# DINT-NSDI24/DINT

Hardware: AMD Instinct MI355X
Metric: Mtxn/s + p50/p99 batch latency, TATP (higher is better)
Workload: dtype u64

## Files before the change

dint_amd/csrc/dint_kv.h:

```cpp
#pragma once
#include <cstdlib>
#include <utility>
#include <vector>

#include "dint_kernels.h"
#include "dint_kv_core.h"
#include "state_block.h"
#include "state_image.h"

#define DINT_KV_MAX_TABLES 5
#define DINT_KV_CTL_BYTES (64 + 24 * KV_NLISTS)
#define DINT_KV_TRACE_WORDS ((size_t)DINT_KV_PMAX * 16 + 16 * 8192)
#define DINT_KV_LOAD_OP 0xF0u

struct kv_dev {
  kv_tab tab[DINT_KV_MAX_TABLES];
  dint_mod mod[DINT_KV_MAX_TABLES];
  dint_mod lockmod[DINT_KV_MAX_TABLES];
  uint32_t gk_base[DINT_KV_MAX_TABLES];
  uint32_t n_tables;
  uint32_t shard_index, shard_count;
  uint32_t same_key;
  uint32_t pass_ins[DINT_KV_MAX_TABLES];
};

struct dint_kv_knobs {
  uint32_t coarse_load = 512;
  uint32_t cap = 0;
  uint32_t lcap = 1024;
  uint32_t cap_mult = 64;
  uint32_t rpt = 0;
  uint32_t no_bm = 0;
  uint32_t hot_min = 0;
  uint32_t no_split = 0;
  uint32_t split_min = 65;
  uint32_t split_target = 384;
  uint32_t one_big_kernel = 0;
  uint32_t workers = 96;
  uint32_t part_first = 0;
  uint32_t sb_split_min = 65;
  uint32_t sb_npmax = 128;
  uint32_t sb_workers = 130;
  uint32_t sb_late_grid = 32;
  uint32_t residency = 0;
  uint32_t no_fuse = 0;
  uint32_t no_ahead = 0;
  uint32_t late_grid = 8;
  uint32_t exp_no_late = 0;
  uint32_t late_fat = 0;
  uint32_t late_big = 0;
};

struct dint_kv {
  uint32_t workload = 0;
  uint32_t n_tables = 0;
  uint32_t val_size = 0;
  int force_rounds = 0;
  uint64_t hash_size[DINT_KV_MAX_TABLES] = {0, 0, 0, 0, 0};
  kv_dev h{};
  kv_dev *d_dev = nullptr;
  uint8_t *d_ctl = nullptr;
  uint64_t *d_trace = nullptr;
  size_t entry_bytes[DINT_KV_MAX_TABLES] = {0, 0, 0, 0, 0};
  dint_kv_knobs knobs;
};

static inline uint32_t dint_kv_cap_mult() {
  const char *v = getenv("DINT_KV_CAP_MULT");
  const unsigned long m = v && *v ? strtoul(v, nullptr, 10) : 64ul;
  return (uint32_t)(m < 2 ? 2 : m > 256 ? 256 : m);
}
int dint_kv_create(dint_kv *kv, uint32_t workload, uint64_t n_rows, dint_shard shard, uint32_t pool_entries = 0,
                   uint32_t flags = 0);
void dint_kv_destroy(dint_kv *kv);
std::vector<std::pair<void *, size_t>> dint_kv_regions(dint_kv *kv);
int64_t dint_kv_dump_rows(dint_kv *kv, uint32_t table, uint64_t *keys, uint32_t *vers, uint8_t *vals, uint64_t cap);
int64_t dint_kv_read_locks(dint_kv *kv, uint32_t table, uint32_t *a, uint32_t *b, uint64_t cap);
struct dint_kv_ahead {
  const void *d_req;
  void *d_rep;
  uint32_t n;
  dint_view view;
};
bool dint_kv_ahead_ok(const dint_kv &kv, int load_mode);
bool dint_kv_one_launch(const dint_kv &kv, int load_mode);
void dint_launch_kv(const void *d_req, void *d_rep, uint32_t n, const dint_kv &kv, dint_log log, dint_scratch s,
                    int load_mode, hipStream_t st, hipEvent_t *ev, const dint_view &view = dint_flat_view(),
                    bool part_done = false, const dint_kv_ahead *next = nullptr);
#define DINT_KV_MULTI_MAX 4u
struct dint_kv_pass {
  const void *d_req;
  void *d_rep;
  uint32_t n;
  const dint_kv *kv;
  dint_log log;
  dint_scratch s;
  dint_view view;
};
void dint_launch_kv_multi(const dint_kv_pass *p, uint32_t n_eng, hipStream_t st, bool part_done = false, const dint_kv_pass *next = nullptr);
bool dint_kv_multi_ahead_ok(const dint_kv &kv);
void dint_launch_home_kv(const void *d_req, uint32_t n, const dint_kv &kv, uint8_t *d_home, hipStream_t st);
struct dint_kv_fmt {
  uint32_t msg, type, table, key, val, ver, val_size;
};
dint_kv_fmt dint_kv_format(uint32_t workload);

struct dint_state_scratch {
  unsigned long long *words;
  uint32_t *blk_cnt;
  uint64_t *blk_off;
  uint32_t nb;
  unsigned long long *digest_part;
};
#define DINT_STATE_DIGEST_GRID 2048u
#define DINT_STATE_WORDS 48u
#define DINT_STATE_DIGEST_AT 16u
uint32_t dint_state_blocks(const dint_kv &kv);
void dint_launch_state_digest(const dint_kv &kv, dint_state_scratch s, hipStream_t st);
void dint_launch_state_diff_count(const dint_kv &a, const dint_kv &b, dint_state_scratch s, hipStream_t st);
void dint_launch_state_diff_write(const dint_kv &a, const dint_kv &b, dint_state_scratch s, void *d_records, uint64_t cap, hipStream_t st);
void dint_launch_state_repair_check(const dint_kv &kv, const void *d_records, uint64_t n, dint_state_scratch s, hipStream_t st);
void dint_launch_state_repair(const dint_kv &kv, const void *d_records, uint64_t n, uint32_t pend_set, dint_dev_stats *stats,
                              dint_state_scratch s, hipStream_t st);

#define DINT_STATE_STATS_GRID 2048u
#define DINT_STATE_STATS_WORDS 80u
struct dint_stats_scratch {
  unsigned long long *part;
// ... 147 lines not shown
```

dint_amd/csrc/k_kv.hip:

```cpp
#include "k_kv_dev.h"

dint_kv_fmt dint_kv_format(uint32_t workload) {
  switch (workload) {
    case DINT_WL_STORE: return {53, 0, 0xFFFFFFFFu, 1, 9, 49, 40};
    case DINT_WL_TATP: return {55, 1, 2, 3, 11, 51, 40};
    default: return {23, 1, 2, 3, 11, 19, 8};
  }
}


static inline uint32_t kv_pick_coarse(uint32_t n, uint32_t load) {
  uint64_t c = ((uint64_t)n + load - 1) / load;
  if (c < 1) c = 1;
  if (c > DINT_KV_CMAX) c = DINT_KV_CMAX;
  return (uint32_t)c;
}
static uint32_t kv_env(const char *name, uint32_t dflt) {
  const char *v = getenv(name);
  return v && *v ? (uint32_t)strtoul(v, nullptr, 10) : dflt;
}
static dint_kv_knobs kv_read_knobs() {
  dint_kv_knobs k;
  k.coarse_load = std::min(8192u, std::max(64u, kv_env("DINT_KV_COARSE_LOAD", KVB_T)));
  k.cap = kv_env("DINT_KV_CAP", 0);
  k.lcap = std::min(KVR_LCAP, kv_env("DINT_KV_LCAP", KVR_LCAP));
  k.cap_mult = dint_kv_cap_mult();
  k.rpt = kv_env("DINT_KV_RPT", 0);
  k.no_bm = kv_env("DINT_KV_NO_BM", 0);
  k.hot_min = kv_env("DINT_KV_HOT_MIN", 0);
  k.no_split = kv_env("DINT_KV_NO_SPLIT", 0);
  k.split_min = std::max(65u, kv_env("DINT_KV_SPLIT_MIN", 65u));
  k.split_target = std::min(448u, std::max(8u, kv_env("DINT_KV_SPLIT_TARGET", 384u)));
  k.one_big_kernel = kv_env("DINT_KV_ONE_BIG_KERNEL", 0);
  k.no_ahead = kv_env("DINT_KV_NO_AHEAD", 0);
  k.no_fuse = kv_env("DINT_KV_NO_FUSE", 0);
  k.sb_split_min = kv_env("DINT_KV_SB_SPLIT_MIN", 65u);
  k.sb_late_grid = std::max(1u, std::min(KVB_GRID, kv_env("DINT_KV_SB_LATE_GRID", 32u)));
  k.sb_npmax = std::max(2u, std::min(KSB_NPMAX, kv_env("DINT_KV_SB_NPMAX", 128u)));
  k.sb_workers = kv_env("DINT_KV_SB_WORKERS", k.sb_npmax + 2u);
  if (k.sb_workers) k.sb_workers = std::max(k.sb_workers, k.sb_npmax + 2u);
  k.workers = std::min(1024u, std::max(KVR_NPMAX + 2u, kv_env("DINT_KV_WORKERS", KVW_GRID)));
  k.part_first = kv_env("DINT_KV_PART_FIRST", 0) & 1u;
  k.late_grid = std::min(KVB_GRID, std::max(1u, kv_env("DINT_KV_LATE_GRID", 8u)));
  k.late_big = kv_env("DINT_KV_LATE_BIG", 0);
  k.exp_no_late = kv_env("DINT_EXP_NO_LATE", 0);
  k.late_fat = kv_env("DINT_KV_LATE_FAT", 0);
  return k;
}

static inline bool kv_uses_hot(const dint_kv &kv, int load_mode) {
  return kv.workload != DINT_WL_SMALLBANK && !(kv.force_rounds & 3) && !load_mode && !kv.knobs.no_split;
}
bool dint_kv_one_launch(const dint_kv &kv, int load_mode) {
  return kv_uses_hot(kv, load_mode) && !kv.knobs.one_big_kernel && !kv.knobs.no_fuse;
}
bool dint_kv_ahead_ok(const dint_kv &kv, int load_mode) {
  if (kv.workload == DINT_WL_SMALLBANK) return !load_mode && !kv.knobs.no_ahead && !kv.knobs.no_fuse;
  return kv_uses_hot(kv, load_mode) && !kv.knobs.one_big_kernel && !kv.knobs.no_ahead;
}

static void kv_fill_pass(kv_pass_args &A, const void *d_req, void *d_rep, uint32_t n, const dint_kv &kv, dint_log log,
                         const dint_scratch &s, int load_mode, const dint_view &view, uint32_t tile) {
  const dint_kv_knobs &K = kv.knobs;
  const uint32_t C = kv_pick_coarse(n, K.coarse_load);
  const uint32_t mean = (n + C - 1) / C;
  uint32_t cap = K.cap_mult * mean + 64;
  cap = std::min(cap, (uint32_t)(s.kbins_slots / C));
  cap = std::max(1u, K.cap ? std::min(cap, K.cap) : cap);
  A.req = (const uint8_t *)d_req; A.rep = (uint8_t *)d_rep; A.n = n;
  A.n_tiles = (n + tile - 1) / tile;
  A.kv = kv.d_dev; A.log = log; A.cut = kv_make_cut(C, n); A.cap = cap;
  A.lcap = K.lcap;
  const uint64_t pn = s.kvs.pass_no;
  A.pno = (uint32_t)(pn & 1u);
  A.bin_cnt = s.kvs.bin_cnt[pn & 1]; A.kbins = s.kvs.kbins[pn & 1]; A.ovl = s.kvs.ovl[pn & 1];
  A.big = s.kvs.ctl[pn % 3]; A.big_z = s.kvs.ctl[(pn + 2) % 3];
  A.blk_pub = s.kvs.pub[pn % 3]; A.blk_pub_z = s.kvs.pub[(pn + 2) % 3];
  A.bigrdy = s.kvs.bigrdy;
  A.ovf = s.ovf; A.ovf2 = s.ovf2; A.stats = s.stats;
  A.bigq = s.bigq;
  A.hotpub = s.hotpub;
  A.lateq = s.lateq;
  A.seq = s.pass_seq ? s.pass_seq : 1u;
  A.inv_n = n > 1 ? (uint32_t)((1ull << 32) / n) : 0xFFFFFFFFu;
  A.load_mode = load_mode;
  A.force_flags = kv.force_rounds | (K.no_bm ? 4 : 0) | (int)(K.hot_min << 8);
  A.split_min = kv_uses_hot(kv, load_mode) ? K.split_min : 0xFFFFFFFFu;
  A.split_target = K.split_target;
  A.np_max = KVR_NPMAX;
  A.sb_pieces = 0;
  A.sbx = s.kvs.sbx;
  if (kv.workload == DINT_WL_SMALLBANK && K.sb_split_min && s.kvs.sbx && !(kv.force_rounds & 3) && !load_mode && !K.no_split) {
    A.split_min = std::max(8u, K.sb_split_min);
    A.np_max = K.sb_npmax;
    A.sb_pieces = 1;
  }
  A.has_log = kv.workload != DINT_WL_STORE;
  A.trace = kv.d_trace;
  A.V = view;
}

extern template int kv_piece_residency<DINT_WL_STORE>(int);
extern template int kv_piece_residency<DINT_WL_TATP>(int);
extern template int kv_piece_residency<DINT_WL_SMALLBANK>(int);
extern template void launch_kv_passes<DINT_WL_STORE>(kv_multi_args &, uint32_t, uint32_t, hipStream_t, hipEvent_t *, const dint_kv_knobs &, bool, const kv_multi_args *, uint32_t);
extern template void launch_kv_passes<DINT_WL_TATP>(kv_multi_args &, uint32_t, uint32_t, hipStream_t, hipEvent_t *, const dint_kv_knobs &, bool, const kv_multi_args *, uint32_t);
extern template void launch_kv_passes<DINT_WL_SMALLBANK>(kv_multi_args &, uint32_t, uint32_t, hipStream_t, hipEvent_t *, const dint_kv_knobs &, bool, const kv_multi_args *, uint32_t);

static inline uint32_t kv_pick_rpt(uint32_t n_total, const dint_kv_knobs &K) {
  if (K.rpt == 1 || K.rpt == 2 || K.rpt == 4) return K.rpt;
  return n_total >= 1024u * 1024u ? 4u : n_total >= 256u * 1024u ? 2u : 1u;
}
static inline uint32_t kv_pick_rpt_ahead(uint32_t n, const dint_kv_knobs &K) {
  if (K.rpt == 4 || (K.rpt == 0 && n >= 256u * 1024u)) return 4u;
  return 2u;
}

static void launch_kv_dispatch(uint32_t workload, kv_multi_args &M, uint32_t n_eng, uint32_t rpt, hipStream_t st, hipEvent_t *ev,
                               const dint_kv_knobs &K, bool part_done = false, const kv_multi_args *next = nullptr, uint32_t next_rpt = 0) {
  switch (workload) {
    case DINT_WL_STORE: launch_kv_passes<DINT_WL_STORE>(M, n_eng, rpt, st, ev, K, part_done, next, next_rpt); break;
    case DINT_WL_TATP: launch_kv_passes<DINT_WL_TATP>(M, n_eng, rpt, st, ev, K, part_done, next, next_rpt); break;
    default: launch_kv_passes<DINT_WL_SMALLBANK>(M, n_eng, rpt, st, ev, K, part_done, next, next_rpt); break;
  }
}

void dint_launch_kv(const void *d_req, void *d_rep, uint32_t n, const dint_kv &kv, dint_log log, dint_scratch s,
                    int load_mode, hipStream_t st, hipEvent_t *ev, const dint_view &view, bool part_done, const dint_kv_ahead *next) {
  if (n == 0) return;
  kv_multi_args M;
  memset(&M, 0, sizeof M);
  const uint32_t rpt = kv_pick_rpt(n, kv.knobs), rpt_a = kv_pick_rpt_ahead(n, kv.knobs);
  kv_fill_pass(M.e[0], d_req, d_rep, n, kv, log, s, load_mode, view, part_done ? KVB_T * rpt_a : KV_TB * rpt);
  kv_multi_args N;
  uint32_t next_rpt = 0;
  if (next && next->n && dint_kv_ahead_ok(kv, load_mode)) {
    dint_scratch sn = s;
    sn.kvs.pass_no = s.kvs.pass_no + 1;
    sn.pass_seq = s.pass_seq + 1 >= 0x3FFFFFFFu ? 1u : s.pass_seq + 1;
    next_rpt = kv_pick_rpt_ahead(next->n, kv.knobs);
    memset(&N, 0, sizeof N);
    kv_fill_pass(N.e[0], next->d_req, next->d_rep, next->n, kv, log, sn, load_mode, next->view, KVB_T * next_rpt);
  } else {
    next = nullptr;
  }
  launch_kv_dispatch(kv.workload, M, 1, rpt, st, ev, kv.knobs, part_done, next ? &N : nullptr, next_rpt);
}

void dint_launch_kv_multi(const dint_kv_pass *p, uint32_t n_eng, hipStream_t st, bool part_done, const dint_kv_pass *next) {
  if (n_eng == 0) return;
  kv_multi_args M, N;
  memset(&M, 0, sizeof M);
  uint32_t n_total = 0;
  for (uint32_t k = 0; k < n_eng; k++) n_total += p[k].n;
  const uint32_t rpt = kv_pick_rpt(n_total, p[0].kv->knobs);
  for (uint32_t k = 0; k < n_eng; k++) kv_fill_pass(M.e[k], p[k].d_req, p[k].d_rep, p[k].n, *p[k].kv, p[k].log, p[k].s, 0, p[k].view, KV_TB * rpt);
  uint32_t next_rpt = 0;
  if (next) {
    uint32_t nmax = 0;
    for (uint32_t k = 0; k < n_eng; k++) nmax = std::max(nmax, next[k].n);
    next_rpt = kv_pick_rpt_ahead(nmax, p[0].kv->knobs);
    memset(&N, 0, sizeof N);
    for (uint32_t k = 0; k < n_eng; k++) {
      dint_scratch sn = next[k].s;
      sn.kvs.pass_no = p[k].s.kvs.pass_no + 1;
      sn.pass_seq = p[k].s.pass_seq + 1 >= 0x3FFFFFFFu ? 1u : p[k].s.pass_seq + 1;
      kv_fill_pass(N.e[k], next[k].d_req, next[k].d_rep, next[k].n, *next[k].kv, next[k].log, sn, 0, next[k].view, KVB_T * next_rpt);
    }
  }
// ... 235 lines not shown
```

dint_amd/csrc/k_kv_dev.h:

```cpp
#pragma once
#include <algorithm>
#include <cstddef>
#include <cstdlib>
#include <cstring>
#include <utility>
#include <vector>

#include "../../include/dint_abi.h"
#include "dint_kv.h"
#define KVB_SORT_INLINE
#include "dint_bins.h"

template <int WL> struct Fmt;
template <> struct Fmt<DINT_WL_STORE> {
  static constexpr uint32_t MSG = 53, TYPE = 0, KEY = 1, VAL = 9, VER = 49, VS = 40;
  static constexpr bool HAS_TABLE = false;
  static constexpr uint32_t TABLE = 0;
};
template <> struct Fmt<DINT_WL_TATP> {
  static constexpr uint32_t MSG = 55, TYPE = 1, KEY = 3, VAL = 11, VER = 51, VS = 40;
  static constexpr bool HAS_TABLE = true;
  static constexpr uint32_t TABLE = 2;
};
template <> struct Fmt<DINT_WL_SMALLBANK> {
// ... 2002 lines not shown
            uint32_t pos;
            if (fancy) {
              const int lw = top(mW & below), lwb = top((mW | mB) & below);
              const uint32_t w = wc + (uint32_t)__popcll(mW & below);
              const uint32_t jj = (lw < 0 ? jc : 0u) + (uint32_t)__popcll(mB & below & above(lw));
              const uint64_t mine = q == 0 ? mA[0] : q == 1 ? mA[1] : q == 2 ? mA[2] : mA[3];
              const bool follows = (mine & below & above(lwb)) != 0 || (lwb < 0 && ((af >> q) & 1u));
              pos = w * stride + (cl == 0 ? 0u : cl == 1 ? 3u * jj + (follows ? 1u : 0u) : cl == 2 ? 3u * jj + 2u : stride - 1u);
            } else {
              pos = 2u * (vc + (uint32_t)__popcll(mV & below)) + (cl ? 1u : 0u);
            }
            if (valid) Rpos[p] = (uint16_t)pos;
            const int tw = top(mW), twb = top(mW | mB);
            wc += (uint32_t)__popcll(mW);
            jc = (tw < 0 ? jc : 0u) + (uint32_t)__popcll(mB & above(tw));
            if (twb >= 0) af = 0;
#pragma unroll
            for (uint32_t i = 0; i < 4; i++) af |= (mA[i] & above(twb)) ? 1u << i : 0u;
            vc += (uint32_t)__popcll(mV);
          }
        }
      }
    }
    __syncthreads();
    for (uint32_t j = 0; j < ntile; j++) {
      const uint32_t p = j * KVB_T + t;
      const uint32_t pos = p < m ? Rpos[p] : 0xFFFFu;
      if (pos != 0xFFFFu) atomicOr(&Rbits[pos >> 5], 1u << (pos & 31));
    }
    {
      uint32_t mx = mylen;
      for (int d = 32; d > 0; d >>= 1) mx = max(mx, (uint32_t)__shfl_xor(mx, d, 64));
      if (lane == 0) Sred[wave] = mx;
      __syncthreads();
      tot = 0;
      for (uint32_t w = 0; w < KVB_W; w++) tot = max(tot, Sred[w]);
    }
    for (uint32_t rw = 0; rw * 32 < tot; rw++) {
      for (uint32_t bits = Rbits[rw]; bits; bits &= bits - 1) {
        const uint32_t r = rw * 32 + (uint32_t)__ffs((int)bits) - 1;
        nrounds++;
        for (uint32_t j = 0; j < ntile; j++) {
          const uint32_t p = j * KVB_T + t;
          if (p < m && Rpos[p] == r) {
            const uint64_t cur = Sk[p];
            const uint32_t gk = kv_cut_gk((uint32_t)(cur >> sh_g), bin, cut), table = kv_table_of(kv, gk);
            kv_do_request<WL>(rep + dint_view_off(V, k_idx(cur), F::MSG), k_type(cur), table, k_q(cur),
                              (uint64_t)(gk - kv->gk_base[table]), kv, stats);
          }
        }
        __builtin_amdgcn_fence(__ATOMIC_SEQ_CST, "workgroup");
        __syncthreads();
      }
    }
    }
    if (wtr && t == 0) { wtr[14] += nrounds; wtr[15] += 1; }
    KVB_STAMP(13);
    __builtin_amdgcn_fence(__ATOMIC_SEQ_CST, "workgroup");
    __syncthreads();
  }
#undef KVB_STAMP
}

#define KVR_LCAP 1024u
#define KVR_F 64u
#define KVR_NPMAX 64u
struct kvr_lds {
  uint4 rec[KVR_LCAP];
  uint32_t hist[KVR_F];
  uint32_t cur[KVR_F];
  uint32_t off[KVR_F + 1];
  uint32_t bigoff[KVR_F];
  uint2 chs[KVR_F];
  uint32_t nch;
  uint32_t cflag[KVR_F];
  uint64_t ckey[KVR_F], hrec[KVR_F];
};
__device__ static inline uint32_t kv_piece_of(uint32_t idx, uint32_t np, uint32_t inv_n) {
  const uint32_t p = (uint32_t)(((uint64_t)idx * np * inv_n) >> 32);
  return p < np ? p : np - 1;
}
#define KVQ_W 3u
enum : uint32_t { KVQ_SUB = 0, KVQ_PIECE = 1, KVQ_REM = 2, KVQ_SOLO = 3 };

__device__ static inline void kv_list_items(const kv_pass_args &A, uint32_t b, const kvr_lds &L, const uint2 *Sbig) {
  const uint32_t t = threadIdx.x & 63u;
  const uint2 bs = Sbig[t];
  uint32_t target = A.split_target;
  if (A.V.seg_cap) {
    uint32_t live = t < A.V.n_seg ? min(A.V.seg_cap, *(const uint32_t *)(A.V.cnt + (size_t)t * A.V.cnt_stride)) : 0u, tot;
    (void)wave_excl_scan_u32(live, &tot);
    if (tot < A.n) target = max(8u, (uint32_t)(((uint64_t)target * max(tot, 1u)) / A.n));
  }
  const uint32_t np0 = (bs.y + target - 1) / target;
  const bool hot = bs.y >= A.split_min && np0 <= A.np_max;
  const uint32_t np = hot ? np0 : 0u;
  const uint32_t nent = bs.y ? (np > 1 ? np + 1 : 1u) : 0u;
  uint32_t tot, at = wave_excl_scan_u32(nent, &tot);
  uint32_t base = 0;
  if (t == 0 && tot) base = atomicAdd(&A.big[3], tot);
  base = (uint32_t)__builtin_amdgcn_readfirstlane((int)base);
  at += base;
  const uint32_t bin = b + A.cut.P * t;
  if (nent && !hot) {
    kv_st_agent(A.bigq + KVQ_W * (size_t)at, make_uint4(bin, bs.x, bs.y, KVQ_SUB));
  } else if (nent) {
    uint64_t hk = L.ckey[t], hr = L.hrec[t];
    if (A.sb_pieces) {
      using F = Fmt<DINT_WL_SMALLBANK>;
      const uint32_t sh_g = 16 + A.cut.ibits;
      uint64_t smp[8];
#pragma unroll
      for (uint32_t j = 0; j < 8; j++) smp[j] = kv_ld_agent(&A.ovf[bs.x + (uint32_t)(((uint64_t)(2 * j + 1) * bs.y) >> 4)]);
      uint32_t best = 0, bj = 0;
#pragma unroll
      for (uint32_t j = 0; j < 8; j++) {
        uint32_t c = 0;
#pragma unroll
        for (uint32_t i = 0; i < 8; i++) c += (smp[i] >> sh_g) == (smp[j] >> sh_g) && pay_q(kv_rec_pay(smp[i])) == pay_q(kv_rec_pay(smp[j]));
        if (c > best) { best = c; bj = j; }
      }
      hr = smp[0];
#pragma unroll
      for (uint32_t j = 1; j < 8; j++) if (j == bj) hr = smp[j];
      const uint32_t hidx = (uint32_t)(hr >> 16) & (uint32_t)((1ull << A.cut.ibits) - 1ull);
      hk = ld_u64(A.rep + dint_view_off(A.V, hidx, F::MSG) + F::KEY);
    }
    for (uint32_t p = 0; p < nent; p++) {
      const uint32_t kind = np == 1 ? KVQ_SOLO : (p < np ? KVQ_PIECE : KVQ_REM);
      uint4 *q = A.bigq + KVQ_W * (size_t)(at + p);
      kv_st_agent(q, make_uint4(bin, bs.x, bs.y, kind | (p << 2) | (np << 10)));
      kv_st_agent(q + 1, make_uint4((uint32_t)hk, (uint32_t)(hk >> 32), at, 0u));
      kv_st_agent(q + 2, make_uint4((uint32_t)hr, (uint32_t)(hr >> 32), 0u, 0u));
    }
  }
  asm volatile("s_waitcnt vmcnt(0)" ::: "memory");
  for (uint32_t p = 0; p < nent; p++)
    if (at + p < DINT_KV_BIGQ_MAX) __hip_atomic_store(&A.bigrdy[at + p], A.seq, __ATOMIC_RELAXED, __HIP_MEMORY_SCOPE_AGENT);
  asm volatile("s_waitcnt vmcnt(0)" ::: "memory");
  if (t == 0) atomicAdd(&A.big[6], 1u);
}

template <int WL, uint32_t NT>
__device__ static inline void kv_coarse_bin(const kv_pass_args &A, const kv_dev *kv, uint32_t coarse, uint8_t *lds_raw,
                                            uint2 *Sbig ,
                                            uint32_t cnt, const uint4 &r0, const uint4 &r1, uint64_t *tr) {
  kvr_lds &L = *(kvr_lds *)lds_raw;
  const uint32_t t = threadIdx.x, lane = t & 63, wave = t >> 6;
  const kv_cut &cut = A.cut;
  const uint32_t C = cut.P, cap = A.cap, sh = 16 + cut.ibits;
  const uint32_t idx_mask = (uint32_t)((1ull << cut.ibits) - 1ull);
  const uint4 *__restrict__ recs = A.kbins + (size_t)coarse * cap;
  if (cnt == 0) {
    if (t == 0) atomicAdd(&A.big[6], 1u);
    return;
  }
  const uint32_t n_in = min(cnt, cap);
  const uint32_t novl = cnt > cap ? A.big[1] : 0u;
  if (t == 0) A.bin_cnt[coarse] = 0;
  auto for_each_record = [&](auto &&f) {
    if (t < n_in) f(r0);
    if (t + NT < n_in) f(r1);
    for (uint32_t k0 = 2 * NT; k0 < n_in; k0 += 8 * NT) {
      uint4 q4[8];
#pragma unroll
      for (uint32_t j = 0; j < 8; j++) {
// ... 277 lines not shown
      if (lane == 0) { H.Lq[q][wave] = ml; H.Aq[q][wave] = ma; }
    }
  }
  __syncthreads();
  uint32_t ev_below = 0, nW = 0;
#pragma unroll
  for (uint32_t wv = 0; wv < KVB_W; wv++) {
    const uint64_t m = H.Bw[wv];
    nW += (uint32_t)__popcll(m);
    ev_below += (uint32_t)__popcll(wv < wave ? m : (wv == wave ? m & lanemask_lt() : 0ull));
  }
  if (H.gbad || nW > KVG_MAXW) return false;
  uint8_t *msg = rep + dint_view_off(V, my_idx, F::MSG);
  for (uint32_t e = 0; e <= nW; e++) {
    if (isR && ev_below == e) {
      kv_hdr Hh;
      kv_hdr_load(Hh, ie);
      const kv_res r = kv_apply<kv_dev_mem>(tb, bucket, Hh, KV_ACT_GET, my_key, msg + F::VAL, 0, blockIdx.x);
      if (r.ok) st_u32(msg + F::VER, r.ver);
      msg[F::TYPE] = (uint8_t)(WL == DINT_WL_STORE ? (r.ok ? 3 : 7) : (r.ok ? 4 : 6));
    }
    __builtin_amdgcn_fence(__ATOMIC_SEQ_CST, "workgroup");
    __syncthreads();
    if (isW && ev_below == e) {
      kv_hdr Hh;
      kv_hdr_load(Hh, ie);
      const uint32_t act = is_set(my_type) ? KV_ACT_SET : is_ins(my_type) ? KV_ACT_INS : KV_ACT_DEL;
      const kv_res r = kv_apply<kv_dev_mem>(tb, bucket, Hh, act, my_key, msg + F::VAL, 0, blockIdx.x);
      uint32_t code;
      if (WL == DINT_WL_STORE) code = my_type == 1 ? (r.ok ? 5 : 7) : 8;
      else code = my_type == 12 ? 15 : my_type == 13 ? 16 : my_type == 18 ? 20 : my_type == 19 ? 21 : my_type == 22 ? 25 : 26;
      if (!r.ok) {
        if (act == KV_ACT_INS) atomicAdd(&stats->pool_exhausted, 1ULL);
        else if (WL != DINT_WL_STORE) atomicAdd(&stats->missing_keys, 1ULL);
      }
      msg[F::TYPE] = (uint8_t)code;
    }
    __builtin_amdgcn_fence(__ATOMIC_SEQ_CST, "workgroup");
    __syncthreads();
  }
  if (WL == DINT_WL_TATP) {
    const uint32_t lockw = H.lockw;
    if (v && (my_type == 1 || my_type == 2)) {
      int last = -1;
#pragma unroll
      for (uint32_t wv = 0; wv < KVB_W; wv++) {
        const uint64_t m = H.Lq[my_q][wv], mb = wv < wave ? m : (wv == wave ? m & lanemask_lt() : 0ull);
        if (mb) last = (int)(wv * 64 + 63 - __clzll((long long)mb));
      }
      const uint32_t seen = last >= 0 ? (uint32_t)((H.Aq[my_q][last >> 6] >> (last & 63)) & 1ull) : (lockw >> (8 * my_q)) & 0xFFu;
      msg[F::TYPE] = (uint8_t)(my_type == 1 ? (seen ? 8 : 7) : 9);
    }
    if (t < 4) {
      int last = -1;
      for (uint32_t wv = 0; wv < KVB_W; wv++)
        if (H.Lq[t][wv]) last = (int)(wv * 64 + 63 - __clzll((long long)H.Lq[t][wv]));
      if (last >= 0) {
        const uint32_t fin = (uint32_t)((H.Aq[t][last >> 6] >> (last & 63)) & 1ull);
        if (fin != ((lockw >> (8 * t)) & 0xFFu)) KV_ST(uint8_t, ie + KV_LOCKB_OFF + t, (uint8_t)fin);
      }
    }
  }
  __builtin_amdgcn_fence(__ATOMIC_SEQ_CST, "workgroup");
  __syncthreads();
  return true;
}
template <int WL>
__device__ __forceinline__ static int kv_solo_item(uint8_t *rep, const kv_cut cut2, const kv_dev *kv, const uint4 d,
                                                   const uint64_t *__restrict__ ovf, uint64_t *__restrict__ ovf2,
                                                   dint_dev_stats *__restrict__ stats, int force_rounds, const dint_view V, uint8_t *lds_raw,
                                                   uint32_t *src, uint32_t *off, uint32_t *cnt, uint64_t *ttr,
                                                   bool preloaded = false ) {
  using F = Fmt<WL>;
  kvh_lds &H = *(kvh_lds *)lds_raw;
  const uint32_t t = threadIdx.x, lane = t & 63, wave = t >> 6;
  const uint32_t h = d.z;
  const uint32_t sh_g = 16 + cut2.ibits, sh_k = 7 + cut2.ibits, idx_mask = (uint32_t)((1ull << cut2.ibits) - 1ull);
  *src = 0; *off = d.y; *cnt = h;
  if (h > KVB_T) return 1;
  auto is_set = [](uint32_t type) -> bool { return WL == DINT_WL_STORE ? type == 1 : (type == 12 || type == 13); };
  auto is_ins = [](uint32_t type) -> bool { return WL == DINT_WL_STORE ? type == 2 : (type == 18 || type == 19); };
  auto is_del = [](uint32_t type) -> bool { return WL == DINT_WL_TATP && (type == 22 || type == 23); };
  __syncthreads();
  if (!preloaded) H.all[t] = t < h ? kv_sort_key(kv_ld_agent(&ovf[d.y + t]), cut2) : ~0ull;
  if (t == 0) { H.bad = 0; H.best = 0; H.bestg = 0; H.dupf = 0; }
  __syncthreads();
  {
    uint32_t N = 64;
    while (N < h) N <<= 1;
    kvb_sort_blocked<1>(H.all, N);
  }
  const uint64_t w = H.all[t];
  const bool valid = t < h;
  const uint64_t prevw = t ? H.all[t - 1] : 0;
  const bool head_k = valid && (t == 0 || (prevw >> sh_k) != (w >> sh_k));
  const bool head_g = valid && (t == 0 || (prevw >> sh_g) != (w >> sh_g));
  const uint64_t mk = __ballot(head_k), mg = __ballot(head_g);
  if (lane == 0) { H.Bw[wave] = mk; H.Bl[wave] = mg; }
  __syncthreads();
  auto next_head = [&](const uint64_t *M) -> uint32_t {
    uint32_t nxt = h;
    for (uint32_t wv = wave; wv < KVB_W && nxt == h; wv++) {
      uint64_t mm = M[wv];
      if (wv == wave) mm &= ~((2ull << lane) - 1ull);
      if (mm) nxt = wv * 64 + (uint32_t)__ffsll((unsigned long long)mm) - 1;
    }
    return nxt;
  };
  if (head_k) atomicMax(&H.best, ((next_head(H.Bw) - t) << 16) | t);
  if (head_g) atomicMax(&H.bestg, ((next_head(H.Bl) - t) << 16) | t);
  __syncthreads();
  const uint32_t L = H.best >> 16, P = H.best & 0xFFFFu;
  uint32_t Gs = H.bestg & 0xFFFFu, Ge = Gs + (H.bestg >> 16);
  if (L > 64) {
    Gs = 0;
    for (uint32_t wv = 0; wv < KVB_W; wv++) {
      uint64_t mm = H.Bl[wv];
      if (wv * 64 > P) break;
      if (wv == (P >> 6)) mm &= (2ull << (P & 63)) - 1ull;
      if (mm) Gs = wv * 64 + 63 - (uint32_t)__clzll((long long)mm);
    }
    Ge = h;
    for (uint32_t wv = P >> 6; wv < KVB_W && Ge == h; wv++) {
      uint64_t mm = H.Bl[wv];
      if (wv == (P >> 6)) mm &= ~((2ull << (P & 63)) - 1ull);
      if (mm) Ge = wv * 64 + (uint32_t)__ffsll((unsigned long long)mm) - 1;
    }
  }
  auto rest = [&](uint32_t lo, uint32_t len) -> int {
    const uint32_t c_rem = h - len;
    if (c_rem == 0) return 0;
    __syncthreads();
    if (valid && (t < lo || t >= lo + len)) H.rem[t < lo ? t : t - len] = w;
    if (t >= c_rem) H.rem[t] = ~0ull;
    __builtin_amdgcn_fence(__ATOMIC_SEQ_CST, "workgroup");
    if (kv_rem_chunks<WL>(rep, cut2, kv, d.x, H.rem, c_rem, H, stats, force_rounds, V, true)) return 0;
    if (ovf2 && t < c_rem) {
      const uint64_t sw = H.rem[t];
      ovf2[d.y + t] = ((sw >> sh_g) << sh_g) | ((uint64_t)((uint32_t)(sw >> 7) & idx_mask) << 16) | ((uint32_t)sw & 0x7Fu) | (((uint32_t)(sw >> sh_k) & 511u) << 7);
    }
    __builtin_amdgcn_fence(__ATOMIC_SEQ_CST, "workgroup");
    *src = 1; *off = d.y; *cnt = c_rem;
    return 1;
  };
  auto phases = [&]() -> int {
    if (!kv_group_phases<WL>(rep, cut2, kv, d.x, H.all, Gs, Ge, H, stats, V)) return 1;
    return rest(Gs, Ge - Gs);
  };
  if (L <= 64) {
    if (ttr && t == 0) ttr[30] = (uint64_t)(d.w & 0xFFFFu) | (1ull << 17) | ((uint64_t)L << 20) | ((uint64_t)h << 32);
    if (Ge - Gs <= 64) return kv_rem_chunks<WL>(rep, cut2, kv, d.x, H.all, h, H, stats, force_rounds, V, true) ? 0 : 1;
    return phases();
  }
  const uint64_t hw = H.all[P];
  const uint32_t hq = pay_q((uint32_t)hw & 0x7Fu);
  const bool v = valid && t >= P && t < P + L;
  const uint32_t my_idx = (uint32_t)(w >> 7) & idx_mask, my_type = valid ? pay_type((uint32_t)w & 0x7Fu) : 0xFFu;
  if (valid && !v && (w >> sh_g) == (hw >> sh_g) && (kv_struct_op<WL>(my_type) || (kv_lock_op<WL>(my_type) && pay_q((uint32_t)w & 0x7Fu) == hq))) atomicOr(&H.bad, kv_struct_op<WL>(my_type) ? 1u : 2u);
  const uint64_t my_key = v ? ld_u64(rep + dint_view_off(V, my_idx, F::MSG) + F::KEY) : 0;
  if (t == P) H.hkey = my_key;
  const bool setop = v && is_set(my_type), insop = v && is_ins(my_type), delop = v && is_del(my_type);
  const bool lk = v && kv_lock_op<WL>(my_type), aq = v && WL == DINT_WL_TATP && my_type == 1;
  if (v && !(kv_simple_op<WL>(my_type) || kv_struct_op<WL>(my_type))) atomicOr(&H.bad, 4u);
  const uint64_t bev = __ballot(setop || insop || delop), bl = __ballot(lk), ba = __ballot(aq), bst = __ballot(insop || delop);
  if (lane == 0) { H.Bw[wave] = bev; H.Bl[wave] = bl; H.Ba[wave] = ba; }
  if (bst && lane == 0) H.dupf = 1;
  H.idx[t] = my_idx;
// ... 194 lines not shown
  const bool locator = t == 0 && c != 0;
  if (locator) {
    const uint32_t gk = kv_cut_gk((uint32_t)(hrec >> sh_g), d.x, cut2);
    table0 = kv_table_of(kv, gk);
    tb0 = kv->tab[table0];
    bucket0 = (uint64_t)(gk - kv->gk_base[table0]);
    kv_hdr_load(Hd, kv_entry_ptr(tb0, bucket0, KV_INLINE));
  }
  __syncthreads();
  if (do_piece) kvb_sort_blocked_u32<1>(H.key, KVB_T);
  if (locator) {
    const kv_where w = kv_locate(tb0, bucket0, Hd, hkey);
    H.found = w.found; H.link = w.link; H.slot = w.slot; H.ver0 = w.ver; H.table = table0;
    H.la0 = WL == DINT_WL_TATP ? (Hd.lockw >> (8 * hq)) & 0xFFu : 0u;
    if (w.found) {
      const uint8_t *rv = kv_entry_ptr(tb0, bucket0, w.link) + KV_VAL_OFF + w.slot * F::VS;
#pragma unroll
      for (uint32_t k = 0; k < F::VS / 4; k++) H.rowv[k] = KV_LD(uint32_t, rv + 4 * k);
    }
  }
  const uint32_t sk = H.key[t];
  const bool v = do_piece && sk != 0xFFFFFFFFu;
  const uint32_t my_idx = sk >> 9, my_type = v ? H.typ[sk & 511u] : 0xFFu;
  if (v && !kv_simple_op<WL>(my_type)) H.bad = 1;
  const bool wr = v && is_writer(my_type), lk = v && kv_lock_op<WL>(my_type), aq = v && WL == DINT_WL_TATP && my_type == 1;
  const uint64_t bw = __ballot(wr), bl = __ballot(lk), ba = __ballot(aq);
  if (lane == 0) { H.Bw[wave] = bw; H.Bl[wave] = bl; H.Ba[wave] = ba; }
  H.idx[t] = my_idx;
  __syncthreads();
  uint32_t wr_below = 0, wr_tot = 0;
  int lw_below = -1, lw_tot = -1, ll_below = -1, ll_tot = -1;
#pragma unroll
  for (uint32_t w = 0; w < KVB_W; w++) {
    const uint64_t mw = H.Bw[w], ml = H.Bl[w];
    const uint64_t mwb = w < wave ? mw : (w == wave ? mw & lanemask_lt() : 0ull), mlb = w < wave ? ml : (w == wave ? ml & lanemask_lt() : 0ull);
    wr_below += (uint32_t)__popcll(mwb); wr_tot += (uint32_t)__popcll(mw);
    if (mwb) lw_below = (int)(w * 64 + 63 - __clzll((long long)mwb));
    if (mw) lw_tot = (int)(w * 64 + 63 - __clzll((long long)mw));
    if (mlb) ll_below = (int)(w * 64 + 63 - __clzll((long long)mlb));
    if (ml) ll_tot = (int)(w * 64 + 63 - __clzll((long long)ml));
  }
  auto acq_at = [&](int p) -> int { return (int)((H.Ba[p >> 6] >> (p & 63)) & 1ull); };
  const unsigned long long mine_w = kvh_word(seq, !H.bad, wr_tot, lw_tot >= 0 ? (int)H.idx[lw_tot] : -1, ll_tot >= 0 ? acq_at(ll_tot) : -1);
  bool all_ok = !H.bad;
  if (nsib > 1 && voting) {
    if (t == 0) __hip_atomic_store(&pub[j], mine_w, __ATOMIC_RELAXED, __HIP_MEMORY_SCOPE_AGENT);
    if (t < nsib) {
      unsigned long long w = 0;
      uint32_t spins = 0;
      for (;;) {
        w = __hip_atomic_load(&pub[t], __ATOMIC_RELAXED, __HIP_MEMORY_SCOPE_AGENT);
        if ((uint32_t)(w >> 34) == (seq & 0x3FFFFFFFu)) break;
        if (++spins > (1u << 22)) { H.timeout = 1; break; }
        __builtin_amdgcn_s_sleep(2);
      }
      H.pub[t] = w;
    }
    __syncthreads();
    if (H.timeout) __builtin_trap();
    for (uint32_t k = 0; k < nsib; k++) all_ok = all_ok && ((H.pub[k] >> 33) & 1ull);
  } else {
    if (t == 0) H.pub[0] = mine_w;
    __syncthreads();
  }
  if (ttr && t == 0) ttr[30] = (uint64_t)(d.w & 0xFFFFu) | ((uint64_t)(all_ok ? 1u : 0u) << 16) | ((uint64_t)(c & 0xFFFu) << 20) | ((uint64_t)c_rem << 32);
  if (!all_ok && voting) {
    if (j != 0 || !do_piece) return 0;
    if (nbr || solo) { *src = 0; *off = d.y; *cnt = h; return 1; }
    const uint32_t nsame = H.nsame;
    __syncthreads();
    if (t == 0) H.nhot = 0;
    __syncthreads();
    for (uint32_t k0 = 0; k0 < h; k0 += KVB_T) {
      const uint32_t k = k0 + t;
      const uint64_t r = k < h ? kv_ld_agent(&ovf[d.y + k]) : 0;
      const bool same = k < h && (r >> sh_g) == (hrec >> sh_g) && pay_kh(kv_rec_pay(r)) == hkh;
      const uint64_t mm = __ballot(same);
      uint32_t at = 0;
      if (lane == 0 && mm) at = atomicAdd(&H.nhot, (uint32_t)__popcll(mm));
      at = (uint32_t)__builtin_amdgcn_readfirstlane((int)at) + (uint32_t)__popcll(mm & lanemask_lt());
      if (same) ovf2[d.y + (h - nsame) + at] = r;
    }
    __builtin_amdgcn_fence(__ATOMIC_SEQ_CST, "workgroup");
    *src = 1; *off = d.y + (h - nsame); *cnt = nsame;
    return 1;
  }
  if (c != 0) {
    uint32_t nw_before = 0, nw_all = 0;
    int lw_before = -1, la_before = -1, jw = -1, jl = -1, la_fin = -1;
    for (uint32_t k = 0; k < np; k++) {
      const unsigned long long w = H.pub[k];
      const uint32_t nwk = (uint32_t)(w >> 23) & 1023u;
      if (k < j) {
        nw_before += nwk;
        if ((w >> 22) & 1ull) lw_before = (int)((w >> 2) & 0xFFFFFu);
        if (w & 2ull) la_before = (int)(w & 1ull);
      }
      nw_all += nwk;
      if (nwk) jw = (int)k;
      if (w & 2ull) { jl = (int)k; la_fin = (int)(w & 1ull); }
    }
    const uint32_t found = H.found, ver0 = H.ver0, la0 = H.la0;
    const kv_tab tb = kv->tab[H.table];
    const uint32_t gk = kv_cut_gk((uint32_t)(hrec >> sh_g), d.x, cut2);
    const uint64_t bucket = (uint64_t)(gk - kv->gk_base[H.table]);
    uint8_t *row = kv_entry_ptr(tb, bucket, H.link) + KV_VAL_OFF + H.slot * F::VS;
    if (v) {
      uint8_t *msg = rep + dint_view_off(V, my_idx, F::MSG);
      uint32_t code;
      bool get = false;
      if (WL == DINT_WL_STORE) {
        code = my_type == 0 ? (found ? 3 : 7) : (found ? 5 : 7);
        get = my_type == 0 && found;
      } else {
        const int seen = ll_below >= 0 ? acq_at(ll_below) : (la_before >= 0 ? la_before : (int)la0);
        switch (my_type) {
          case 0: code = found ? 4 : 6; get = found != 0; break;
          case 1: code = seen ? 8 : 7; break;
          case 2: code = 9; break;
          case 12: code = 15; break;
          default: code = 16; break;
        }
      }
      if (get) {
        const int widx = lw_below >= 0 ? (int)H.idx[lw_below] : lw_before;
        if (widx >= 0) {
          kv_copy_words(msg + F::VAL, rep + dint_view_off(V, (uint32_t)widx, F::MSG) + F::VAL, F::VS);
        } else {
#pragma unroll
          for (uint32_t k = 0; k < F::VS / 4; k++) st_u32(msg + F::VAL + 4 * k, H.rowv[k]);
        }
        st_u32(msg + F::VER, ver0 + nw_before + wr_below);
      }
      msg[F::TYPE] = (uint8_t)code;
    }
    if (found && nw_all && (int)j == jw && (int)t == lw_tot) {
      kv_copy_words(row, rep + dint_view_off(V, my_idx, F::MSG) + F::VAL, F::VS);
      KV_ST(uint32_t, &kv_entry_hdr(tb, bucket, H.link)->ver[H.slot], ver0 + nw_all);
    }
    if (WL == DINT_WL_TATP && t == 0) {
      if ((int)j == jl && la_fin >= 0 && (uint32_t)la_fin != la0) KV_ST(uint8_t, kv_entry_ptr(tb, bucket, KV_INLINE) + KV_LOCKB_OFF + hq, (uint8_t)la_fin);
      if (!found && wr_tot) atomicAdd(&stats->missing_keys, (unsigned long long)wr_tot);
    }
  }
  if (c_rem == 0) return 0;
  __builtin_amdgcn_fence(__ATOMIC_SEQ_CST, "workgroup");
  if (c_rem <= KVB_T && kv_rem_chunks<WL>(rep, cut2, kv, d.x, H.rem, c_rem, H, stats, force_rounds, V)) return 0;
  __builtin_amdgcn_fence(__ATOMIC_SEQ_CST, "workgroup");
  *src = 1; *off = d.y; *cnt = c_rem;
  return 1;
}

template <int WL>
__device__ __forceinline__ static void kv_serial_group(uint8_t *rep, const kv_cut cut2, const kv_dev *kv, uint32_t bin, const uint64_t *R, uint32_t Gs,
                                                       uint32_t Ge, kvh_lds &H, dint_dev_stats *__restrict__ stats, const dint_view V) {
  using F = Fmt<WL>;
  const uint32_t t = threadIdx.x, n = Ge - Gs;
  const uint32_t sh_g = 16 + cut2.ibits, idx_mask = (uint32_t)((1ull << cut2.ibits) - 1ull);
  __syncthreads();
  {
    const uint64_t w = t < n ? R[Gs + t] : 0;
    const uint32_t idx = (uint32_t)(w >> 7) & idx_mask, pay = (uint32_t)w & 0x7Fu;
    H.key[t] = t < n ? (idx << 9) | t : 0xFFFFFFFFu;
    H.typ[t] = (uint8_t)(pay_type(pay) & 0xFFu);
    H.qq[t] = (uint8_t)pay_q(pay);
  }
  __syncthreads();
// ... 366 lines not shown
    *src = 0; *off = d.y; *cnt = h;
    return 1;
  }
  const uint32_t solo_rem = solo ? H.nrem : 0u;
  auto done = [&]() -> int {
    if (!solo_rem) return 0;
    __builtin_amdgcn_fence(__ATOMIC_SEQ_CST, "workgroup");
    *src = 1; *off = d.y; *cnt = solo_rem;
    return 1;
  };
  if (t < KVB_W) H.G[t] = kv_ld_agent(&sbx[(size_t)(first + j) * KSB_WORDS + 4 * KVB_W + t]);
  if (t < np) H.pub[t] = __hip_atomic_load(&pub[t], __ATOMIC_RELAXED, __HIP_MEMORY_SCOPE_AGENT);
  __syncthreads();
  if (c == 0) return done();
  uint32_t nw_before = 0, nw_all = 0;
  int lw_before = -1, jw = -1;
  for (uint32_t k = 0; k < np; k++) {
    const unsigned long long w = H.pub[k];
    const uint32_t nwk = (uint32_t)(w >> 23) & 1023u;
    if (k < j) {
      nw_before += nwk;
      if ((w >> 22) & 1ull) lw_before = (int)((w >> 2) & 0xFFFFFu);
    }
    nw_all += nwk;
    if (nwk) jw = (int)k;
  }
  const uint32_t found = H.found, ver0 = H.ver0;
  uint32_t miss = 0;
  if (v && !foreign) {
    const bool granted = (H.G[wave] >> lane) & 1ull;
    uint32_t code;
    bool get = false;
    switch (my_type) {
      case 0: code = granted ? 7 : 8; get = granted; break;
      case 1: code = granted ? 9 : 10; get = granted; break;
      case 2: code = 11; break;
      case 3: code = 12; break;
      case 4: code = 13; miss = !found; break;
      case 5: code = 14; miss = !found; break;
      default: code = 18; get = true; break;
    }
    if (get && found) {
      const int widx = lw_below >= 0 ? (int)H.idx[lw_below] : lw_before;
      if (widx >= 0) {
        const uint8_t *fm = rep + dint_view_off(V, (uint32_t)widx, F::MSG) + F::VAL;
        const uint32_t a0 = ld_u32(fm), a1 = ld_u32(fm + 4);
        st_u32(msg + F::VAL, a0); st_u32(msg + F::VAL + 4, a1);
      } else {
        st_u32(msg + F::VAL, H.rowv[0]); st_u32(msg + F::VAL + 4, H.rowv[1]);
      }
      st_u32(msg + F::VER, ver0 + nw_before + wr_below);
    } else if (get && my_type != 17u) {
      miss = 1;
    }
    msg[F::TYPE] = (uint8_t)code;
  }
  {
    const uint64_t mm = __ballot(miss != 0);
    if (lane == 0 && mm) atomicAdd(&stats->missing_keys, (unsigned long long)__popcll(mm));
  }
  if (found && nw_all && (int)j == jw && (int)t == lw_tot) {
    uint8_t *row = kv_entry_ptr(tb, bucket, H.link) + KV_VAL_OFF + H.slot * F::VS;
    KV_ST(uint32_t, row, ld_u32(msg + F::VAL));
    KV_ST(uint32_t, row + 4, ld_u32(msg + F::VAL + 4));
    KV_ST(uint32_t, &kv_entry_hdr(tb, bucket, H.link)->ver[H.slot], ver0 + nw_all);
  }
  return done();
}

static_assert(sizeof(kvb_lds) + KVB_BM_BYTES + sizeof(kv_dev) <= 160 * 1024, "k_kv_big must fit the 160 KB of LDS of a gfx950 CU");
static_assert(sizeof(kvb_lds) + (KV_HOT_BM ? KV_HOT_BM_W * 10 : 16) + sizeof(kv_dev) <= 160 * 1024, "k_kv_big must fit the 160 KB of LDS of a gfx950 CU");
#define KVW_GRID 96u
template <int WL>
__device__ __forceinline__ static void kv_hot_role(const kv_pass_args &A, kv_dev &Skv, uint8_t *Lraw, uint32_t &Stk, uint32_t bx, uint32_t by) {
  const uint32_t t = threadIdx.x;
  if (t < sizeof(kv_dev) / 4) ((uint32_t *)&Skv)[t] = kv_dev_word(A.kv, A.big, t);
  __syncthreads();
  kv_dev_pend_set(Skv, A.pno);
  kv_cut cut2 = A.cut;
  cut2.P = A.cut.P * KVR_F;
  uint64_t *tr = A.trace ? A.trace + 2048 * 32 + 32 * (size_t)(by * KVB_GRID + bx) : nullptr;
  for (bool first = true;; first = false) {
    __syncthreads();
    if (t == 0) {
      const uint32_t i = atomicAdd(&A.big[4], 1u);
      uint32_t got = KV_NONE;
      for (uint32_t spins = 0; i < DINT_KV_BIGQ_MAX; spins++) {
        if (__hip_atomic_load(&A.bigrdy[i], __ATOMIC_RELAXED, __HIP_MEMORY_SCOPE_AGENT) == A.seq) { got = i; break; }
        if (__hip_atomic_load(&A.big[6], __ATOMIC_RELAXED, __HIP_MEMORY_SCOPE_AGENT) >= A.cut.P &&
            i >= __hip_atomic_load(&A.big[3], __ATOMIC_RELAXED, __HIP_MEMORY_SCOPE_AGENT)) break;
        if (spins > (1u << 22)) __builtin_trap();
        __builtin_amdgcn_s_sleep(4);
      }
      Stk = got;
    }
    __syncthreads();
    const uint32_t i = Stk;
    if (i == KV_NONE) break;
    const uint4 d = kv_ld_agent(A.bigq + KVQ_W * (size_t)i);
    uint32_t src = 0, off = d.y, cnt = d.z;
    uint64_t *ttr = first ? tr : nullptr;
    if (ttr && t == 0) { ttr[0] = __builtin_amdgcn_s_memrealtime(); ttr[2] = d.z; ttr[3] = d.x; ttr[30] = d.w; }
    int run = 1;
    if constexpr (WL == DINT_WL_SMALLBANK) {
      if ((d.w & 3u) != KVQ_SUB)
        run = kv_sb_item<WL>(A.rep, cut2, &Skv, d, kv_ld_agent(A.bigq + KVQ_W * (size_t)i + 1), kv_ld_agent(A.bigq + KVQ_W * (size_t)i + 2), A.ovf, A.ovf2,
                             A.hotpub, A.sbx, A.seq, A.inv_n, A.stats, A.V, Lraw, &src, &off, &cnt);
      if (run && src == 1 && cnt <= KVB_T) {
        kvh_lds &Hh = *(kvh_lds *)Lraw;
        __syncthreads();
        Hh.rem[t] = t < cnt ? A.ovf2[off + t] : 0ull;
        if (kv_rem_chunks<WL>(A.rep, cut2, &Skv, d.x, Hh.rem, cnt, Hh, A.stats, A.force_flags & 1, A.V)) run = 0;
      }
      if (run && t == 0) A.lateq[atomicAdd(&A.big[5], 1u)] = make_uint4(d.x, off, cnt, src);
    } else {
    if ((d.w & 3u) == KVQ_SOLO)
      run = kv_solo_item<WL>(A.rep, cut2, &Skv, d, A.ovf, A.ovf2, A.stats, A.force_flags & 1, A.V, Lraw, &src, &off, &cnt, ttr);
    else if ((d.w & 3u) != KVQ_SUB)
      run = kv_hot_item<WL>(A.rep, cut2, &Skv, d, kv_ld_agent(A.bigq + KVQ_W * (size_t)i + 1), kv_ld_agent(A.bigq + KVQ_W * (size_t)i + 2), A.ovf, A.ovf2,
                            A.hotpub, A.seq, A.inv_n, A.stats, A.force_flags & 1, A.V, Lraw, &src, &off, &cnt, ttr);
    if (run && t == 0) {
      A.lateq[atomicAdd(&A.big[5], 1u)] = make_uint4(d.x, off, cnt, src);
      atomicAdd(&A.stats->late_requests, (unsigned long long)cnt);
      atomicAdd(&A.stats->late_items[(d.w & 3u) == KVQ_SUB ? 0 : (d.w & 3u) == KVQ_SOLO ? 1 : 2], 1ULL);
    }
    }
    if (ttr && t == 0) ttr[1] = __builtin_amdgcn_s_memrealtime();
  }
}
template <int WL>
__global__ void __launch_bounds__(KVB_T, 4) k_kv_hot(kv_multi_args M) {
  __shared__ kv_dev Skv;
  __shared__ __attribute__((aligned(16))) uint8_t Lraw[sizeof(kvh_lds)];
  __shared__ uint32_t Stk;
  const kv_pass_args &A = M.e[blockIdx.y];
  if (blockIdx.x >= A.big[3]) return;
  kv_hot_role<WL>(A, Skv, Lraw, Stk, blockIdx.x, blockIdx.y);
}

template <int WL, int RPT>
__global__ void __launch_bounds__(KVB_T, 4) k_kv_hot_part(kv_pass_args H, kv_pass_args P) {
  constexpr size_t LB = sizeof(kvh_lds) > sizeof(kv_part_lds<RPT, KVB_T>) ? sizeof(kvh_lds) : sizeof(kv_part_lds<RPT, KVB_T>);
  __shared__ kv_dev Skv;
  __shared__ __attribute__((aligned(16))) uint8_t Lraw[LB];
  __shared__ uint32_t Stk;
  if (blockIdx.x < KVB_GRID) {
    if (blockIdx.x < H.big[3]) kv_hot_role<WL>(H, Skv, Lraw, Stk, blockIdx.x, 0);
    return;
  }
  const uint32_t b = blockIdx.x - KVB_GRID;
  if (b >= P.n_tiles) return;
  kv_part_body<WL, RPT, KVB_T>(P, *(kv_part_lds<RPT, KVB_T> *)Lraw, b == 0);
}

template <int WL, int RPT>
__global__ void __launch_bounds__(KVB_T, 4) k_kv_pass(kv_multi_args M, uint32_t n_eng, uint32_t sum_c, kv_multi_args PM ,
                                                       uint32_t max_tiles ,
                                                       uint32_t n_work ,
                                                       uint32_t part_first ) {
  constexpr size_t LW = sizeof(kvs_lds) > sizeof(kvh_lds) ? sizeof(kvs_lds) : sizeof(kvh_lds);
  constexpr size_t L1 = LW > sizeof(kvr_lds) ? LW : sizeof(kvr_lds);
  constexpr size_t LB = L1 > sizeof(kv_part_lds<RPT ? RPT : 1, KVB_T>) ? L1 : sizeof(kv_part_lds<RPT ? RPT : 1, KVB_T>);
  __shared__ kv_dev Skv;
  __shared__ __attribute__((aligned(16))) uint8_t Lraw[LB];
  __shared__ uint2 Sbig[KVR_F];
  __shared__ uint32_t Stk;
  uint32_t b = blockIdx.x;
  if (b < sum_c) {
    uint32_t e = 0;
    while (e + 1 < n_eng && b >= M.e[e].cut.P) { b -= M.e[e].cut.P; e++; }
    kv_resolve_role<WL>(M.e[e], b, Skv, Lraw, Sbig);
    return;
  }
  b -= sum_c;
  const uint32_t nw = n_work * n_eng, nt = RPT != 0 ? max_tiles * n_eng : 0u;
  const bool worker = part_first ? b >= nt : b < nw;
  if (worker) {
    if (part_first) b -= nt;
    if (b >= nw) return;
    const uint32_t e = b / n_work;
    kv_hot_role<WL>(M.e[e], Skv, Lraw, Stk, b - e * n_work, e);
    return;
  }
  if constexpr (RPT != 0) {
    if (!part_first) b -= nw;
    if (b >= nt) return;
    const uint32_t e = b / max_tiles, slot = b - e * max_tiles;
    const kv_pass_args &P = PM.e[e];
    if (slot >= P.n_tiles) return;
    kv_part_body<WL, RPT, KVB_T>(P, *(kv_part_lds<RPT, KVB_T> *)Lraw, slot == 0);
  }
}

template <int WL>
__global__ void __launch_bounds__(KVB_T, 1) k_kv_big(kv_multi_args M, uint32_t from_late) {
  static_assert(sizeof(kv_dev) + sizeof(kvb_lds) + (WL == DINT_WL_SMALLBANK ? KVB_BM_BYTES : 16) + 64 <= 160 * 1024, "k_kv_big's LDS must fit a gfx950 compute unit");
  __shared__ kv_dev Skv;
  __shared__ __attribute__((aligned(16))) uint8_t Lraw[sizeof(kvb_lds)];
  __shared__ __attribute__((aligned(16))) uint8_t Lbm[WL == DINT_WL_SMALLBANK ? KVB_BM_BYTES : KV_HOT_BM ? KV_HOT_BM_W * 10 : 16];
  __shared__ uint32_t Stk;
  const kv_pass_args &A = M.e[blockIdx.y];
  const uint32_t nq = from_late ? A.big[5] : A.big[3];
  if (blockIdx.x >= nq) return;
  const uint32_t t = threadIdx.x;
  if (t < sizeof(kv_dev) / 4) ((uint32_t *)&Skv)[t] = kv_dev_word(A.kv, A.big, t);
  __syncthreads();
  kv_dev_pend_set(Skv, A.pno);
// ... 122 lines not shown
```

Before: 3056.

## Carry leftover hot-item work back into same block instead of late queue

When a hot item leaves a small remainder (src==1, at most one tile), the hot worker rewrites the queue entry as a carried SOLO item and processes it again itself, up to a bounded number of turns, rather than pushing it to the late queue. The goal is to avoid late-kernel round trips and the latency of deferred work. The solo path now reads from ovf2 for carried entries, and the src code for the same-key tail changes from 1 to 2. This adds extra per-block iterations and state encoded in the high bits of Stk. It can be disabled with DINT_KV_NO_CARRY.

After: 3036. Within noise of the previous version (-0.7%).

```diff
diff --git a/dint_amd/csrc/dint_kv.h b/dint_amd/csrc/dint_kv.h
--- a/dint_amd/csrc/dint_kv.h
+++ b/dint_amd/csrc/dint_kv.h
@@ -44,6 +44,7 @@
   uint32_t sb_late_grid = 32;
   uint32_t residency = 0;
   uint32_t no_fuse = 0;
+  uint32_t no_carry = 0;
   uint32_t no_ahead = 0;
   uint32_t late_grid = 8;
   uint32_t exp_no_late = 0;
diff --git a/dint_amd/csrc/k_kv.hip b/dint_amd/csrc/k_kv.hip
--- a/dint_amd/csrc/k_kv.hip
+++ b/dint_amd/csrc/k_kv.hip
@@ -34,6 +34,7 @@
   k.one_big_kernel = kv_env("DINT_KV_ONE_BIG_KERNEL", 0);
   k.no_ahead = kv_env("DINT_KV_NO_AHEAD", 0);
   k.no_fuse = kv_env("DINT_KV_NO_FUSE", 0);
+  k.no_carry = kv_env("DINT_KV_NO_CARRY", 0);
   k.sb_split_min = kv_env("DINT_KV_SB_SPLIT_MIN", 65u);
   k.sb_late_grid = std::max(1u, std::min(KVB_GRID, kv_env("DINT_KV_SB_LATE_GRID", 32u)));
   k.sb_npmax = std::max(2u, std::min(KSB_NPMAX, kv_env("DINT_KV_SB_NPMAX", 128u)));
@@ -84,7 +85,7 @@
   A.seq = s.pass_seq ? s.pass_seq : 1u;
   A.inv_n = n > 1 ? (uint32_t)((1ull << 32) / n) : 0xFFFFFFFFu;
   A.load_mode = load_mode;
-  A.force_flags = kv.force_rounds | (K.no_bm ? 4 : 0) | (int)(K.hot_min << 8);
+  A.force_flags = kv.force_rounds | (K.no_bm ? 4 : 0) | (K.no_carry ? 8 : 0) | (int)(K.hot_min << 8);
   A.split_min = kv_uses_hot(kv, load_mode) ? K.split_min : 0xFFFFFFFFu;
   A.split_target = K.split_target;
   A.np_max = KVR_NPMAX;
diff --git a/dint_amd/csrc/k_kv_dev.h b/dint_amd/csrc/k_kv_dev.h
--- a/dint_amd/csrc/k_kv_dev.h
+++ b/dint_amd/csrc/k_kv_dev.h
@@ -2108,6 +2108,9 @@
 }
 #define KVQ_W 3u
 enum : uint32_t { KVQ_SUB = 0, KVQ_PIECE = 1, KVQ_REM = 2, KVQ_SOLO = 3 };
+#define KVQ_CARRY 0x80000000u
+#define KVW_AGAIN 0x80000000u
+#define KVQ_CARRY_MAX 8u
 
 __device__ static inline void kv_list_items(const kv_pass_args &A, uint32_t b, const kvr_lds &L, const uint2 *Sbig) {
   const uint32_t t = threadIdx.x & 63u;
@@ -2551,7 +2554,7 @@
   auto is_ins = [](uint32_t type) -> bool { return WL == DINT_WL_STORE ? type == 2 : (type == 18 || type == 19); };
   auto is_del = [](uint32_t type) -> bool { return WL == DINT_WL_TATP && (type == 22 || type == 23); };
   __syncthreads();
-  if (!preloaded) H.all[t] = t < h ? kv_sort_key(kv_ld_agent(&ovf[d.y + t]), cut2) : ~0ull;
+  if (!preloaded) H.all[t] = t < h ? kv_sort_key(kv_ld_agent(&((d.w & KVQ_CARRY) ? (const uint64_t *)ovf2 : ovf)[d.y + t]), cut2) : ~0ull;
   if (t == 0) { H.bad = 0; H.best = 0; H.bestg = 0; H.dupf = 0; }
   __syncthreads();
   {
@@ -2912,7 +2915,7 @@
       if (same) ovf2[d.y + (h - nsame) + at] = r;
     }
     __builtin_amdgcn_fence(__ATOMIC_SEQ_CST, "workgroup");
-    *src = 1; *off = d.y + (h - nsame); *cnt = nsame;
+    *src = 2; *off = d.y + (h - nsame); *cnt = nsame;
     return 1;
   }
   if (c != 0) {
@@ -3445,7 +3448,7 @@
   uint64_t *tr = A.trace ? A.trace + 2048 * 32 + 32 * (size_t)(by * KVB_GRID + bx) : nullptr;
   for (bool first = true;; first = false) {
     __syncthreads();
-    if (t == 0) {
+    if (t == 0 && (WL == DINT_WL_SMALLBANK || first || !(Stk & KVW_AGAIN))) {
       const uint32_t i = atomicAdd(&A.big[4], 1u);
       uint32_t got = KV_NONE;
       for (uint32_t spins = 0; i < DINT_KV_BIGQ_MAX; spins++) {
@@ -3458,8 +3461,8 @@
       Stk = got;
     }
     __syncthreads();
-    const uint32_t i = Stk;
-    if (i == KV_NONE) break;
+    const uint32_t i = WL == DINT_WL_SMALLBANK ? Stk : Stk & ~KVW_AGAIN;
+    if (Stk == KV_NONE) break;
     const uint4 d = kv_ld_agent(A.bigq + KVQ_W * (size_t)i);
     uint32_t src = 0, off = d.y, cnt = d.z;
     uint64_t *ttr = first ? tr : nullptr;
@@ -3482,10 +3485,21 @@
     else if ((d.w & 3u) != KVQ_SUB)
       run = kv_hot_item<WL>(A.rep, cut2, &Skv, d, kv_ld_agent(A.bigq + KVQ_W * (size_t)i + 1), kv_ld_agent(A.bigq + KVQ_W * (size_t)i + 2), A.ovf, A.ovf2,
                             A.hotpub, A.seq, A.inv_n, A.stats, A.force_flags & 1, A.V, Lraw, &src, &off, &cnt, ttr);
-    if (run && t == 0) {
-      A.lateq[atomicAdd(&A.big[5], 1u)] = make_uint4(d.x, off, cnt, src);
-      atomicAdd(&A.stats->late_requests, (unsigned long long)cnt);
-      atomicAdd(&A.stats->late_items[(d.w & 3u) == KVQ_SUB ? 0 : (d.w & 3u) == KVQ_SOLO ? 1 : 2], 1ULL);
+    if (t == 0) {
+      const uint32_t turns = (d.w >> 24) & 15u, kind = d.w & 3u;
+      const uint32_t tk = Stk & ~KVW_AGAIN;
+      if (run && !(A.force_flags & 8) && src == 1 && cnt <= KVB_T && turns < KVQ_CARRY_MAX) {
+        kv_st_agent(A.bigq + KVQ_W * (size_t)tk, make_uint4(d.x, off, cnt, KVQ_SOLO | KVQ_CARRY | ((turns + 1u) << 24)));
+        asm volatile("s_waitcnt vmcnt(0)" ::: "memory");
+        Stk = tk | KVW_AGAIN;
+      } else {
+        if (d.w & KVQ_CARRY) Stk = tk;
+        if (run) {
+          A.lateq[atomicAdd(&A.big[5], 1u)] = make_uint4(d.x, off, cnt, d.w & KVQ_CARRY ? 1u : src);
+          atomicAdd(&A.stats->late_requests, (unsigned long long)cnt);
+          atomicAdd(&A.stats->late_items[kind == KVQ_SUB ? 0 : kind == KVQ_SOLO ? 1 : 2], 1ULL);
+        }
+      }
     }
     }
     if (ttr && t == 0) ttr[1] = __builtin_amdgcn_s_memrealtime();
```
